# DataTunerX/datatunerx

Measured on AMD Instinct MI355X. Metric: tokens_per_sec_llama2_7b_lora_sft, higher is better.
Workload: dtype bf16; 1 GPU; model=llama2-7b, global_batch=64, seq_len=1024, parallelism=dp1, finetuning_type=lora

## Files before the change

datatunerx_amd/ops/hip/attn_bwd.hip:

```cpp
#include "dtx_common.h"

typedef __attribute__((ext_vector_type(16))) float f32x16;
typedef __attribute__((ext_vector_type(4))) unsigned int u32x4;

#define MFMA32(a, b, c) __builtin_amdgcn_mfma_f32_32x32x16_bf16(a, b, c, 0, 0, 0)
#define NEG_INF (-3.0e38f)
#define LOG2E 1.4426950408889634f

__device__ __forceinline__ unsigned bw_cvt_pk_bf16(float lo, float hi) {
  unsigned r;
  asm volatile("v_cvt_pk_bf16_f32 %0, %1, %2\n\ts_nop 1"
               : "=v"(r) : "v"(lo), "v"(hi));
  return r;
}

__device__ __forceinline__ int bw_crow(int r, int hi) {
  return (r & 3) + 8 * (r >> 2) + 4 * hi;
}

typedef __attribute__((ext_vector_type(4))) __bf16 bf16x4;
#define DTX_AS3 __attribute__((address_space(3)))
template <int STRIDE>
__device__ __forceinline__ short8v tr_bfrag(
    const DTX_AS3 unsigned short* img, int k0, int n0, int lane) {
  const int row = k0 + ((lane >> 2) & 3);
  const int col = n0 + ((lane >> 4) & 1) * 16 + (lane & 3) * 4;
  const DTX_AS3 unsigned short* p = img + row * STRIDE + col;
  union { bf16x4 v[2]; short8v s; } u;
  u.v[0] = __builtin_amdgcn_ds_read_tr16_b64_v4bf16(
      (DTX_AS3 bf16x4*)p);
  u.v[1] = __builtin_amdgcn_ds_read_tr16_b64_v4bf16(
      (DTX_AS3 bf16x4*)(p + 4 * STRIDE));
  return u.s;
}

__device__ __forceinline__ void conv_c_to_frag(const f32x16& p,
                                               short8v& f0, short8v& f1) {
  unsigned c0 = bw_cvt_pk_bf16(p[0], p[1]);
  unsigned c1 = bw_cvt_pk_bf16(p[2], p[3]);
  unsigned c2 = bw_cvt_pk_bf16(p[4], p[5]);
  unsigned c3 = bw_cvt_pk_bf16(p[6], p[7]);
  unsigned c4 = bw_cvt_pk_bf16(p[8], p[9]);
  unsigned c5 = bw_cvt_pk_bf16(p[10], p[11]);
  unsigned c6 = bw_cvt_pk_bf16(p[12], p[13]);
  unsigned c7 = bw_cvt_pk_bf16(p[14], p[15]);
  auto r02 = __builtin_amdgcn_permlane32_swap(c0, c2, false, false);
  auto r13 = __builtin_amdgcn_permlane32_swap(c1, c3, false, false);
  auto r46 = __builtin_amdgcn_permlane32_swap(c4, c6, false, false);
  auto r57 = __builtin_amdgcn_permlane32_swap(c5, c7, false, false);
  u32x4 lo{(unsigned)r02[0], (unsigned)r13[0],
           (unsigned)r02[1], (unsigned)r13[1]};
  u32x4 hi4{(unsigned)r46[0], (unsigned)r57[0],
            (unsigned)r46[1], (unsigned)r57[1]};
  f0 = *reinterpret_cast<short8v*>(&lo);
  f1 = *reinterpret_cast<short8v*>(&hi4);
}

template <int D>
__global__ __launch_bounds__(DTX_BLOCK)
void attn_delta2_kernel(const unsigned short* __restrict__ dO,
                        const unsigned short* __restrict__ O,
                        float* __restrict__ delta,
                        long nrows, int H, int S) {
  constexpr int LPR = D / 8;
  constexpr int RPW = 64 / LPR;
  const int lane = threadIdx.x & 63;
  const int wid = threadIdx.x >> 6;
  const int sub = lane / LPR;
  const int g = lane % LPR;
  for (long r0 = ((long)blockIdx.x * 4 + wid) * RPW; r0 < nrows;
       r0 += (long)gridDim.x * 4 * RPW) {
    const long row = r0 + sub;
    float acc = 0.f;
    if (row < nrows) {
      const long base = row * D + g * 8;
      float a[8], b8[8];
      load_bf16x8(dO + base, a);
      load_bf16x8(O + base, b8);
#pragma unroll
      for (int i = 0; i < 8; ++i) acc += a[i] * b8[i];
    }
#pragma unroll
    for (int off = LPR / 2; off > 0; off >>= 1)
      acc += __shfl_xor(acc, off, 64);
    if (g == 0 && row < nrows) {
      const int h = (int)(row % H);
      const long bs = row / H;
      const int s = (int)(bs % S);
      const long b = bs / S;
      delta[((long)b * H + h) * S + s] = acc;
    }
  }
}

template <int D>
struct DkdvLds {
  unsigned short Qr[2][64][D + 8];
  unsigned short dOr[2][64][D + 8];
};

template <int D>
__global__ __launch_bounds__(512, 1)
void attn_bwd_dkdv2_kernel(const unsigned short* __restrict__ Q,
                           const unsigned short* __restrict__ Kp,
                           const unsigned short* __restrict__ Vp,
                           const unsigned short* __restrict__ dO,
                           const float* __restrict__ lse_in,
                           const float* __restrict__ delta_in,
                           unsigned short* __restrict__ dK,
                           unsigned short* __restrict__ dV,
                           int B, int Hq, int Hkv, int S, int Skv,
                           float scale, int causal) {
  constexpr int DC16 = D / 16;
  constexpr int ND32 = D / 32;
  __shared__ DkdvLds<D> lds;
  __shared__ float lsed[2][64 + 64];

  const int lane = threadIdx.x & 63;
  const int wid = threadIdx.x >> 6;
  const int l31 = lane & 31;
  const int hi = lane >> 5;
  const int rep = Hq / Hkv;
  const bool role_dv = wid < 4;

  const int bh = blockIdx.y;
  const int b = bh / Hkv, hkv = bh % Hkv;
  const int kv0b = blockIdx.x * 128;
  const int kw = kv0b + (wid & 3) * 32;

  const int qrowstr = Hq * D, krowstr = Hkv * D;
  const long kbase = (long)b * Skv * krowstr + (long)hkv * D;
  const int diag = Skv - S;
  const float kscale = scale * LOG2E;

  short8v kfrag[DC16], vfrag[DC16];
  {
    const int krow = kw + l31;
#pragma unroll
    for (int kc = 0; kc < DC16; ++kc) {
      kfrag[kc] = short8v{0, 0, 0, 0, 0, 0, 0, 0};
      vfrag[kc] = short8v{0, 0, 0, 0, 0, 0, 0, 0};
      if (krow < Skv) {
        const long off = kbase + (long)krow * krowstr + kc * 16 + hi * 8;
        kfrag[kc] = *reinterpret_cast<const short8v*>(Kp + off);
        if (!role_dv)
          vfrag[kc] = *reinterpret_cast<const short8v*>(Vp + off);
      }
    }
  }

  f32x16 acc[ND32];
#pragma unroll
  for (int c = 0; c < ND32; ++c)
#pragma unroll
    for (int r = 0; r < 16; ++r) acc[c][r] = 0.f;

  for (int gi = 0; gi < rep; ++gi) {
    const int hq = hkv * rep + gi;
    const long qbase = (long)b * S * qrowstr + (long)hq * D;
    const long lbase = ((long)b * Hq + hq) * S;

    const int qs_lo = causal ? max(0, (kv0b - diag) / 64) : 0;
    const int qs_hi = (S + 63) / 64;
    constexpr int RIT = (64 * (D / 8)) / 512;
    short8v stg[RIT * 2];
    auto issue_stage = [&](int qs) {
#pragma unroll
      for (int it = 0; it < RIT; ++it) {
        const int idx = threadIdx.x + it * 512;
        const int row = idx / (D / 8), g = idx % (D / 8);
        const int q0s = qs * 64;
        short8v q8 = {0, 0, 0, 0, 0, 0, 0, 0};
        short8v d8 = {0, 0, 0, 0, 0, 0, 0, 0};
        if (q0s + row < S) {
          const long off = qbase + (long)(q0s + row) * qrowstr + g * 8;
          q8 = *reinterpret_cast<const short8v*>(Q + off);
          d8 = *reinterpret_cast<const short8v*>(dO + off);
        }
        stg[it * 2] = q8;
        stg[it * 2 + 1] = d8;
      }
    };
    auto write_stage = [&](int slot) {
#pragma unroll
      for (int it = 0; it < RIT; ++it) {
        const int idx = threadIdx.x + it * 512;
        const int row = idx / (D / 8), g = idx % (D / 8);
        *reinterpret_cast<short8v*>(&lds.Qr[slot][row][g * 8]) =
            stg[it * 2];
        *reinterpret_cast<short8v*>(&lds.dOr[slot][row][g * 8]) =
            stg[it * 2 + 1];
      }
    };
    auto write_lsed = [&](int slot, int qs) {
      if (threadIdx.x < 64) {
        const int qg = qs * 64 + threadIdx.x;
        lsed[slot][threadIdx.x] = qg < S ? lse_in[lbase + qg] : 0.f;
        lsed[slot][64 + threadIdx.x] =
            qg < S ? delta_in[lbase + qg] : 0.f;
      }
    };
    int cur = 0;
    if (qs_lo < qs_hi) {
      issue_stage(qs_lo);
      write_stage(0);
      write_lsed(0, qs_lo);
      __syncthreads();
    }
    for (int qs = qs_lo; qs < qs_hi; ++qs) {
      const int q0s = qs * 64;
      if (qs + 1 < qs_hi) issue_stage(qs + 1);

#pragma unroll
      for (int qh = 0; qh < 2; ++qh) {
      const int q0 = q0s + qh * 32;
      const int qoff = qh * 32;
      const bool live_tile =
          !(q0 >= S || (causal && (q0 + 31 + diag < kw)));
      if (live_tile) {

      f32x16 sv, dpv;
#pragma unroll
      for (int r = 0; r < 16; ++r) { sv[r] = 0.f; dpv[r] = 0.f; }
      if (role_dv) {
#pragma unroll
        for (int kc = 0; kc < DC16; ++kc) {
          short8v qa = *reinterpret_cast<const short8v*>(
              &lds.Qr[cur][qoff + l31][kc * 16 + hi * 8]);
          sv = MFMA32(qa, kfrag[kc], sv);
        }
      } else {
#pragma unroll
        for (int kc = 0; kc < DC16; ++kc) {
          short8v qa = *reinterpret_cast<const short8v*>(
              &lds.Qr[cur][qoff + l31][kc * 16 + hi * 8]);
          short8v da = *reinterpret_cast<const short8v*>(
              &lds.dOr[cur][qoff + l31][kc * 16 + hi * 8]);
          sv = MFMA32(qa, kfrag[kc], sv);
          dpv = MFMA32(da, vfrag[kc], dpv);
        }
      }

      const int kvg = kw + l31;
      const bool interior = (kv0b + 128 <= Skv) && (q0 + 32 <= S) &&
                            (!causal || (kw + 31 <= q0 + diag));
#pragma unroll
      for (int r = 0; r < 16; ++r) {
        const int qg = q0 + bw_crow(r, hi);
        const float lse2 = lsed[cur][qoff + bw_crow(r, hi)] * LOG2E;
        const float dlt = lsed[cur][64 + qoff + bw_crow(r, hi)];
        float p;
        if (interior) {
          p = __builtin_exp2f(sv[r] * kscale - lse2);
        } else {
          const bool dead = (kvg >= Skv) | (qg >= S) |
                            (causal && (kvg > qg + diag));
          p = dead ? 0.f : __builtin_exp2f(sv[r] * kscale - lse2);
        }
        sv[r] = p;
        dpv[r] = p * (dpv[r] - dlt) * scale;
      }

      short8v f0, f1;
      if (role_dv) conv_c_to_frag(sv, f0, f1);
      else conv_c_to_frag(dpv, f0, f1);
      const DTX_AS3 unsigned short* img3 = role_dv
          ? (const DTX_AS3 unsigned short*)&lds.dOr[cur][0][0]
          : (const DTX_AS3 unsigned short*)&lds.Qr[cur][0][0];
#pragma unroll
      for (int c = 0; c < ND32; ++c) {
        short8v b0 = tr_bfrag<D + 8>(img3, qoff + hi * 8, c * 32, lane);
        short8v b1 = tr_bfrag<D + 8>(img3, qoff + 16 + hi * 8, c * 32,
                                     lane);
        acc[c] = MFMA32(f0, b0, acc[c]);
        acc[c] = MFMA32(f1, b1, acc[c]);
        __builtin_amdgcn_sched_barrier(0);
      }
      }
      }
      if (qs + 1 < qs_hi) {
        write_stage(cur ^ 1);
        write_lsed(cur ^ 1, qs + 1);
      }
      __syncthreads();
      cur ^= 1;
    }
  }

  unsigned short* out = role_dv ? dV : dK;
#pragma unroll
  for (int r = 0; r < 16; ++r) {
    const int kvg = kw + bw_crow(r, hi);
    if (kvg < Skv) {
      unsigned short* orow = out + kbase + (long)kvg * krowstr;
#pragma unroll
      for (int c = 0; c < ND32; ++c)
        orow[c * 32 + l31] = f2bf(acc[c][r]);
    }
  }
}

template <int D>
struct DqLds {
  unsigned short K[2][128][D + 8];
  unsigned short V[2][128][D + 8];
};

template <int D>
__global__ __launch_bounds__(512, 1)
void attn_bwd_dq2_kernel(const unsigned short* __restrict__ Q,
                         const unsigned short* __restrict__ Kp,
                         const unsigned short* __restrict__ Vp,
                         const unsigned short* __restrict__ dO,
                         const float* __restrict__ lse_in,
                         const float* __restrict__ delta_in,
                         unsigned short* __restrict__ dQ,
                         int B, int Hq, int Hkv, int S, int Skv,
                         float scale, int causal) {
  constexpr int KVB = 64;
  constexpr int DC16 = D / 16;
  constexpr int ND32 = D / 32;
  __shared__ DqLds<D> lds;

  const int lane = threadIdx.x & 63;
  const int wid = threadIdx.x >> 6;
  const int l31 = lane & 31;
  const int hi = lane >> 5;

  const int bh = blockIdx.y;
  const int b = bh / Hq, hq = bh % Hq;
  const int hkv = hq / (Hq / Hkv);
  const int q0 = blockIdx.x * 256;
  const int qw = q0 + wid * 32;

  const int qrowstr = Hq * D, krowstr = Hkv * D;
  const long qbase = (long)b * S * qrowstr + (long)hq * D;
  const long kbase = (long)b * Skv * krowstr + (long)hkv * D;
  const long lbase = ((long)b * Hq + hq) * S;
  const int diag = Skv - S;
  const float kscale = scale * LOG2E;

  short8v qfrag[DC16], dofrag[DC16];
  float lse2 = 0.f, dlt = 0.f;
  {
    const int qrow = qw + l31;
    if (qrow < S) {
#pragma unroll
      for (int kc = 0; kc < DC16; ++kc) {
        const long off = qbase + (long)qrow * qrowstr + kc * 16 + hi * 8;
        qfrag[kc] = *reinterpret_cast<const short8v*>(Q + off);
        dofrag[kc] = *reinterpret_cast<const short8v*>(dO + off);
      }
      lse2 = lse_in[lbase + qrow] * LOG2E;
      dlt = delta_in[lbase + qrow];
    } else {
#pragma unroll
      for (int kc = 0; kc < DC16; ++kc) {
        qfrag[kc] = short8v{0, 0, 0, 0, 0, 0, 0, 0};
        dofrag[kc] = short8v{0, 0, 0, 0, 0, 0, 0, 0};
      }
    }
  }

  f32x16 dq_acc[ND32];
#pragma unroll
  for (int c = 0; c < ND32; ++c)
#pragma unroll
    for (int r = 0; r < 16; ++r) dq_acc[c][r] = 0.f;

  const int q_hi_blk = min(q0 + 255, S - 1);
  const int kv_hi = causal ? min(Skv - 1, q_hi_blk + diag) : (Skv - 1);
  const int nstages = kv_hi / 128 + 1;

  constexpr int KIT = (128 * (D / 8)) / 512;
  short8v stg[KIT * 2];
  auto issue_stage = [&](int st2) {
    const int kvs = st2 * 128;
#pragma unroll
    for (int it = 0; it < KIT; ++it) {
      const int idx = threadIdx.x + it * 512;
      const int row = idx / (D / 8), g = idx % (D / 8);
      short8v k8 = {0, 0, 0, 0, 0, 0, 0, 0};
      short8v v8 = {0, 0, 0, 0, 0, 0, 0, 0};
      if (kvs + row < Skv) {
        const long off = kbase + (long)(kvs + row) * krowstr + g * 8;
        k8 = *reinterpret_cast<const short8v*>(Kp + off);
        v8 = *reinterpret_cast<const short8v*>(Vp + off);
      }
      stg[it * 2] = k8;
      stg[it * 2 + 1] = v8;
    }
  };
  auto write_stage = [&](int slot) {
#pragma unroll
    for (int it = 0; it < KIT; ++it) {
      const int idx = threadIdx.x + it * 512;
      const int row = idx / (D / 8), g = idx % (D / 8);
      *reinterpret_cast<short8v*>(&lds.K[slot][row][g * 8]) =
          stg[it * 2];
      *reinterpret_cast<short8v*>(&lds.V[slot][row][g * 8]) =
          stg[it * 2 + 1];
    }
  };
  issue_stage(0);
  write_stage(0);
  __syncthreads();
  int cur = 0;
  for (int st2 = 0; st2 < nstages; ++st2) {
    if (st2 + 1 < nstages) issue_stage(st2 + 1);
    const int kvs = st2 * 128;

    for (int kh = 0; kh < 2; ++kh) {
    const int kv0 = kvs + kh * KVB;
    const int koff = kh * KVB;
    const bool wave_dead = (kv0 > kv_hi) ||
                           (causal && (kv0 > qw + 31 + diag));
    if (!wave_dead) {
      const int qg = qw + l31;
      const bool interior = (kv0 + KVB <= Skv) &&
                            (!causal || (kv0 + KVB - 1 <= qw + diag));
#pragma unroll
      for (int ss = 0; ss < 2; ++ss) {
        f32x16 st, dpt;
#pragma unroll
        for (int r = 0; r < 16; ++r) { st[r] = 0.f; dpt[r] = 0.f; }
#pragma unroll
        for (int kc = 0; kc < DC16; ++kc) {
          short8v ka = *reinterpret_cast<const short8v*>(
              &lds.K[cur][koff + ss * 32 + l31][kc * 16 + hi * 8]);
          short8v va = *reinterpret_cast<const short8v*>(
              &lds.V[cur][koff + ss * 32 + l31][kc * 16 + hi * 8]);
          st = MFMA32(ka, qfrag[kc], st);
          dpt = MFMA32(va, dofrag[kc], dpt);
        }
        f32x16 dst;
#pragma unroll
        for (int r = 0; r < 16; ++r) {
          float p;
          if (interior) {
            p = __builtin_exp2f(st[r] * kscale - lse2);
          } else {
            const int kvg = kv0 + ss * 32 + bw_crow(r, hi);
            const bool dead = (kvg >= Skv) | (qg >= S) |
                              (causal && (kvg > qg + diag));
            p = dead ? 0.f : __builtin_exp2f(st[r] * kscale - lse2);
          }
          dst[r] = p * (dpt[r] - dlt) * scale;
        }
        short8v f0, f1;
        conv_c_to_frag(dst, f0, f1);
        const DTX_AS3 unsigned short* k3 =
            (const DTX_AS3 unsigned short*)&lds.K[cur][0][0];
#pragma unroll
        for (int c = 0; c < ND32; ++c) {
          short8v kt0 = tr_bfrag<D + 8>(k3, koff + ss * 32 + hi * 8,
                                        c * 32, lane);
          dq_acc[c] = MFMA32(f0, kt0, dq_acc[c]);
        }
        __builtin_amdgcn_sched_barrier(0);
#pragma unroll
        for (int c = 0; c < ND32; ++c) {
          short8v kt1 = tr_bfrag<D + 8>(k3, koff + ss * 32 + 16 + hi * 8,
                                        c * 32, lane);
          dq_acc[c] = MFMA32(f1, kt1, dq_acc[c]);
        }
        __builtin_amdgcn_sched_barrier(0);
      }
    }
    }
    if (st2 + 1 < nstages) write_stage(cur ^ 1);
    __syncthreads();
    cur ^= 1;
  }

#pragma unroll
  for (int r = 0; r < 16; ++r) {
    const int qg = qw + bw_crow(r, hi);
    if (qg < S) {
      unsigned short* qrow = dQ + qbase + (long)qg * qrowstr;
#pragma unroll
      for (int c = 0; c < ND32; ++c)
        qrow[c * 32 + l31] = f2bf(dq_acc[c][r]);
    }
  }
}

void launch_attn_delta(const void* dO, const void* O, float* delta,
                       long nrows, int H, int S, int D, hipStream_t st) {
  const int rpw = 64 / (D / 8);
  long gw = DTX_CDIV(nrows, 4 * rpw);
  int grid = (int)(gw < 2048 ? (gw < 1 ? 1 : gw) : 2048);
  if (D == 128) {
    attn_delta2_kernel<128><<<grid, DTX_BLOCK, 0, st>>>(
        (const unsigned short*)dO, (const unsigned short*)O, delta,
        nrows, H, S);
  } else if (D == 64) {
    attn_delta2_kernel<64><<<grid, DTX_BLOCK, 0, st>>>(
        (const unsigned short*)dO, (const unsigned short*)O, delta,
        nrows, H, S);
  }
}

void launch_attn_bwd_dkdv(const void* q, const void* k, const void* v,
                          const void* dO, const float* lse,
                          const float* delta, void* dk, void* dv, int B,
                          int Hq, int Hkv, int S, int Skv, int D,
                          float scale, int causal, hipStream_t st) {
  dim3 grid(DTX_CDIV(Skv, 128), B * Hkv);
  if (D == 128) {
    attn_bwd_dkdv2_kernel<128><<<grid, 512, 0, st>>>(
        (const unsigned short*)q, (const unsigned short*)k,
        (const unsigned short*)v, (const unsigned short*)dO,
        lse, delta, (unsigned short*)dk, (unsigned short*)dv,
        B, Hq, Hkv, S, Skv, scale, causal);
  } else if (D == 64) {
    attn_bwd_dkdv2_kernel<64><<<grid, 512, 0, st>>>(
        (const unsigned short*)q, (const unsigned short*)k,
        (const unsigned short*)v, (const unsigned short*)dO,
        lse, delta, (unsigned short*)dk, (unsigned short*)dv,
        B, Hq, Hkv, S, Skv, scale, causal);
  }
}

void launch_attn_bwd_dq(const void* q, const void* k, const void* v,
                        const void* dO, const float* lse,
                        const float* delta, void* dq, int B, int Hq,
                        int Hkv, int S, int Skv, int D, float scale,
                        int causal, hipStream_t st) {
  dim3 grid(DTX_CDIV(S, 256), B * Hq);
  if (D == 128) {
    attn_bwd_dq2_kernel<128><<<grid, 512, 0, st>>>(
        (const unsigned short*)q, (const unsigned short*)k,
        (const unsigned short*)v,
        (const unsigned short*)dO, lse, delta, (unsigned short*)dq,
        B, Hq, Hkv, S, Skv, scale, causal);
  } else if (D == 64) {
    attn_bwd_dq2_kernel<64><<<grid, 512, 0, st>>>(
        (const unsigned short*)q, (const unsigned short*)k,
        (const unsigned short*)v,
        (const unsigned short*)dO, lse, delta, (unsigned short*)dq,
        B, Hq, Hkv, S, Skv, scale, causal);
  }
}
```

datatunerx_amd/ops/hip/bindings.cpp:

```cpp
#include <torch/extension.h>
#include <ATen/cuda/CUDAContext.h>
#include <hip/hip_runtime.h>

void launch_rmsnorm_fwd(const void*, const void*, void*, float*, int, int,
                        float, hipStream_t);
int rmsnorm_bwd_nblocks(int M);
void launch_rmsnorm_bwd(const void*, const void*, const void*, const float*,
                        const void*, void*, float*, float*, int, int,
                        hipStream_t);
void launch_rope(const void*, const float*, const float*, void*, long, int,
                 int, int, int, int, const int*, int, hipStream_t);
void launch_swiglu_fwd(const void*, const void*, void*, long, hipStream_t);
void launch_swiglu_bwd(const void*, const void*, const void*, void*, void*,
                       long, hipStream_t);
void launch_xent_fwd(const void*, const long*, float*, float*, long, int,
                     long, hipStream_t);
void launch_xent_bwd(const void*, const long*, const float*, const float*,
                     void*, long, int, long, hipStream_t);
void launch_dequant_int8(const void*, const float*, void*, long, int,
                         hipStream_t);
void launch_dequant_int4(const void*, const float*, void*, long, int, int,
                         hipStream_t);
void launch_xent_lse_merge(const void*, const long*, float*, float*,
                           float*, long, int, long, long, hipStream_t);
void launch_xent_dlogits(const void*, const long*, const float*, void*,
                         long, int, long, long, hipStream_t);
void launch_adamw(void*, float*, const float*, float*, float*, long, float,
                  float, float, float, float, int, hipStream_t);
void launch_l2_norm(const float*, float*, float*, long, hipStream_t);
int lora_contract_ksplit(int K, long M);
void launch_dropout_mask(void*, long, unsigned long long, float,
                         hipStream_t);
void launch_lora_contract(const void*, const void*, const void*, float*,
                          float*, long, int, int, unsigned long long,
                          float, hipStream_t);
void launch_lora_expand_add(void*, const float*, const void*, const void*,
                            long, int, int, float, unsigned long long,
                            float, hipStream_t);
int lora_wgrad_splitm(int K, int r, long M);
void launch_lora_wgrad(const float*, const void*, const void*, float*,
                       float*, long, int, int, float, unsigned long long,
                       float, hipStream_t);
void launch_attn_fwd(const void*, const void*, const void*, void*, float*,
                     int, int, int, int, int, int, float, int, hipStream_t);
void launch_transpose_sd(const void*, void*, int, int, int, int,
                         hipStream_t);
int attn_decode_nsplit(int Skv);
void launch_gemv_bf16(const void*, const void*, void*, int, int,
                      hipStream_t);
void launch_qgemv_int8(const void*, const void*, const float*, void*, int,
                       int, int, hipStream_t);
void launch_qgemv_int4(const void*, const void*, const float*, void*, int,
                       int, int, int, hipStream_t);
void launch_mlora_shrink(const void*, const void*, const int*, float*, int,
                         int, int, int, hipStream_t);
void launch_mlora_expand_add(void*, const float*, const void*, const float*,
                             const int*, int, int, int, int, hipStream_t);
void launch_gemm_nt(const void*, const void*, const void*, void*, long,
                    int, int, hipStream_t);
void launch_attn_decode(const void*, const void*, const void*,
                        const int*, float*, void*, float*, int, int, int,
                        int, int, float, int, hipStream_t);
void launch_attn_delta(const void*, const void*, float*, long, int, int,
                       int, hipStream_t);
void launch_attn_bwd_dkdv(const void*, const void*, const void*,
                          const void*, const float*, const float*,
                          void*, void*, int, int, int, int, int, int,
                          float, int, hipStream_t);
void launch_attn_bwd_dq(const void*, const void*, const void*,
                        const void*, const float*, const float*, void*,
                        int, int, int, int, int, int, float, int,
                        hipStream_t);

namespace {

hipStream_t cur_stream() {
  return (hipStream_t)at::cuda::getCurrentCUDAStream().stream();
}

void check_bf16_contig(const torch::Tensor& t, const char* name) {
  TORCH_CHECK(t.is_cuda(), name, " must be on GPU");
  TORCH_CHECK(t.scalar_type() == torch::kBFloat16, name, " must be bf16");
  TORCH_CHECK(t.is_contiguous(), name, " must be contiguous");
}

std::vector<torch::Tensor> rmsnorm_fwd(torch::Tensor x, torch::Tensor w,
                                       double eps) {
  check_bf16_contig(x, "x");
  check_bf16_contig(w, "w");
  const int H = (int)x.size(-1);
  const long M = x.numel() / H;
  TORCH_CHECK(H % 8 == 0, "H % 8");
  auto y = torch::empty_like(x);
  auto inv = torch::empty({M}, x.options().dtype(torch::kFloat));
  launch_rmsnorm_fwd(x.data_ptr(), w.data_ptr(), y.data_ptr(),
                     inv.data_ptr<float>(), (int)M, H, (float)eps,
                     cur_stream());
  return {y, inv};
}

std::vector<torch::Tensor> rmsnorm_bwd(torch::Tensor dy, torch::Tensor x,
                                       torch::Tensor w, torch::Tensor inv,
                                       c10::optional<torch::Tensor> dres) {
  check_bf16_contig(dy, "dy");
  check_bf16_contig(x, "x");
  const int H = (int)x.size(-1);
  const long M = x.numel() / H;
  auto dx = torch::empty_like(x);
  auto dw = torch::empty({H}, x.options().dtype(torch::kFloat));
  const int nb = rmsnorm_bwd_nblocks((int)M);
  auto part = torch::empty({nb, H}, x.options().dtype(torch::kFloat));
  const void* drp = nullptr;
  if (dres.has_value()) {
    check_bf16_contig(*dres, "dres");
    TORCH_CHECK(dres->numel() == x.numel(), "dres shape");
    drp = dres->data_ptr();
  }
  launch_rmsnorm_bwd(dy.data_ptr(), x.data_ptr(), w.data_ptr(),
                     inv.data_ptr<float>(), drp, dx.data_ptr(),
                     part.data_ptr<float>(), dw.data_ptr<float>(), (int)M, H,
                     cur_stream());
  return {dx, dw};
}

torch::Tensor rope(torch::Tensor x, torch::Tensor cosb, torch::Tensor sinb,
                   long pos0, bool backward,
                   c10::optional<torch::Tensor> pos_dev) {
  check_bf16_contig(x, "x");
  TORCH_CHECK(x.dim() == 4, "x must be [B,S,H,D]");
  TORCH_CHECK(cosb.scalar_type() == torch::kFloat && cosb.is_contiguous());
  const int B = (int)x.size(0), S = (int)x.size(1), H = (int)x.size(2),
            D = (int)x.size(3);
  TORCH_CHECK(D % 8 == 0, "D % 8");
  const int* pd = nullptr;
  int pos_per_b = 0;
  if (pos_dev.has_value()) {
    TORCH_CHECK(pos_dev->scalar_type() == torch::kInt &&
                pos_dev->is_cuda(), "pos_dev must be int32 on GPU");
    pd = pos_dev->data_ptr<int>();
    pos_per_b = pos_dev->numel() > 1;
    if (pos_per_b)
      TORCH_CHECK(pos_dev->numel() == B, "pos_dev must be [1] or [B]");
    TORCH_CHECK(cosb.size(0) >= S, "rope table too short");
  } else {
    TORCH_CHECK(cosb.size(0) >= pos0 + S, "rope table too short");
  }
  auto y = torch::empty_like(x);
  launch_rope(x.data_ptr(), cosb.data_ptr<float>(), sinb.data_ptr<float>(),
              y.data_ptr(), B, S, H, D, (int)pos0, backward ? 1 : 0, pd,
              pos_per_b, cur_stream());
  return y;
}

torch::Tensor swiglu_fwd(torch::Tensor gate, torch::Tensor up) {
  check_bf16_contig(gate, "gate");
  check_bf16_contig(up, "up");
  TORCH_CHECK(gate.numel() % 8 == 0);
  auto out = torch::empty_like(gate);
  launch_swiglu_fwd(gate.data_ptr(), up.data_ptr(), out.data_ptr(),
                    gate.numel(), cur_stream());
  return out;
}

std::vector<torch::Tensor> swiglu_bwd(torch::Tensor dout, torch::Tensor gate,
                                      torch::Tensor up) {
  check_bf16_contig(dout, "dout");
  auto dg = torch::empty_like(gate);
  auto du = torch::empty_like(up);
  launch_swiglu_bwd(dout.data_ptr(), gate.data_ptr(), up.data_ptr(),
                    dg.data_ptr(), du.data_ptr(), gate.numel(),
                    cur_stream());
  return {dg, du};
}

std::vector<torch::Tensor> xent_fwd(torch::Tensor logits,
                                    torch::Tensor targets, long ignore) {
  check_bf16_contig(logits, "logits");
  TORCH_CHECK(targets.scalar_type() == torch::kLong);
  const int V = (int)logits.size(-1);
  const long N = logits.numel() / V;
  TORCH_CHECK(V % 8 == 0, "V % 8");
  auto loss = torch::empty({N}, logits.options().dtype(torch::kFloat));
  auto lse = torch::empty({N}, logits.options().dtype(torch::kFloat));
  launch_xent_fwd(logits.data_ptr(), targets.data_ptr<long>(),
                  loss.data_ptr<float>(), lse.data_ptr<float>(), N, V,
                  ignore, cur_stream());
  return {loss, lse};
}

torch::Tensor xent_bwd(torch::Tensor logits, torch::Tensor targets,
                       torch::Tensor lse, torch::Tensor dloss, long ignore) {
  check_bf16_contig(logits, "logits");
  const int V = (int)logits.size(-1);
  const long N = logits.numel() / V;
  auto dlogits = torch::empty_like(logits);
  launch_xent_bwd(logits.data_ptr(), targets.data_ptr<long>(),
                  lse.data_ptr<float>(), dloss.data_ptr<float>(),
                  dlogits.data_ptr(), N, V, ignore, cur_stream());
  return dlogits;
}

static const void* opt_mask(const c10::optional<torch::Tensor>& m,
                            long numel, const char* name) {
  if (!m.has_value()) return nullptr;
  check_bf16_contig(*m, name);
  TORCH_CHECK(m->numel() == numel, name, " shape mismatch");
  return m->data_ptr();
}

torch::Tensor lora_contract(torch::Tensor x, torch::Tensor w,
                            c10::optional<torch::Tensor> mask,
                            int64_t seed, double keep) {
  check_bf16_contig(x, "x");
  check_bf16_contig(w, "w");
  const int K = (int)x.size(-1);
  const long M = x.numel() / K;
  const int r = (int)w.size(0);
  TORCH_CHECK(w.size(1) == K, "w [r,K] mismatch");
  TORCH_CHECK(r <= 64, "r <= 64");
  TORCH_CHECK(K % 8 == 0);
  auto t = torch::empty({M, r}, x.options().dtype(torch::kFloat));
  const int nsplit = lora_contract_ksplit(K, M);
  torch::Tensor part;
  float* part_ptr = nullptr;
  if (nsplit > 1) {
    part = torch::empty({nsplit, M, r}, x.options().dtype(torch::kFloat));
    part_ptr = part.data_ptr<float>();
  }
  launch_lora_contract(x.data_ptr(), w.data_ptr(),
                       opt_mask(mask, x.numel(), "mask"), part_ptr,
                       t.data_ptr<float>(), M, K, r,
                       (unsigned long long)seed, (float)keep,
                       cur_stream());
  return t;
}

void lora_expand_add(torch::Tensor y, torch::Tensor t, torch::Tensor w,
                     double scale, c10::optional<torch::Tensor> mask,
                     int64_t seed, double keep) {
  check_bf16_contig(y, "y");
  check_bf16_contig(w, "w");
  const int N = (int)y.size(-1);
  const long M = y.numel() / N;
  const int r = (int)w.size(1);
  TORCH_CHECK(w.size(0) == N, "w [N,r] mismatch");
  TORCH_CHECK(t.scalar_type() == torch::kFloat && t.is_contiguous());
  auto wt = w.t().contiguous();
  TORCH_CHECK(keep >= 1.0 || (r <= 16 && N % 8 == 0 && M >= 64),
              "RNG dropout needs the r<=16 fast path; materialize the "
              "mask for this shape");
  launch_lora_expand_add(y.data_ptr(), t.data_ptr<float>(), wt.data_ptr(),
                         opt_mask(mask, y.numel(), "mask"), M, N, r,
                         (float)scale, (unsigned long long)seed,
                         (float)keep, cur_stream());
}

torch::Tensor lora_wgrad(torch::Tensor t, torch::Tensor x, double scale,
                         c10::optional<torch::Tensor> mask,
                         int64_t seed, double keep) {
  check_bf16_contig(x, "x");
  TORCH_CHECK(t.scalar_type() == torch::kFloat && t.is_contiguous());
  const int K = (int)x.size(-1);
  const long M = x.numel() / K;
  const int r = (int)t.size(-1);
  auto out = torch::empty({r, K}, x.options().dtype(torch::kFloat));
  const int sm = lora_wgrad_splitm(K, r, M);
  auto part = torch::empty({sm, r, K}, x.options().dtype(torch::kFloat));
  launch_lora_wgrad(t.data_ptr<float>(), x.data_ptr(),
                    opt_mask(mask, x.numel(), "mask"),
                    part.data_ptr<float>(), out.data_ptr<float>(), M, K, r,
                    (float)scale, (unsigned long long)seed, (float)keep,
                    cur_stream());
  return out;
}

torch::Tensor dropout_mask(int64_t M, int64_t K, int64_t seed, double keep,
                           torch::Tensor like) {
  TORCH_CHECK((M * K) % 8 == 0, "M*K % 8 == 0");
  auto m = torch::empty({M, K}, like.options().dtype(torch::kBFloat16));
  launch_dropout_mask(m.data_ptr(), M * K, (unsigned long long)seed,
                      (float)keep, cur_stream());
  return m;
}

void adamw(torch::Tensor p, torch::Tensor master, torch::Tensor grad,
           torch::Tensor m, torch::Tensor v, double lr, double b1, double b2,
           double eps, double wd, long step) {
  check_bf16_contig(p, "p");
  TORCH_CHECK(master.scalar_type() == torch::kFloat);
  TORCH_CHECK(grad.scalar_type() == torch::kFloat);
  TORCH_CHECK(p.numel() % 4 == 0, "flat param buffer must be padded to 4");
  launch_adamw(p.data_ptr(), master.data_ptr<float>(),
               grad.data_ptr<float>(), m.data_ptr<float>(),
               v.data_ptr<float>(), p.numel(), (float)lr, (float)b1,
               (float)b2, (float)eps, (float)wd, (int)step, cur_stream());
}

torch::Tensor l2_norm(torch::Tensor x) {
  TORCH_CHECK(x.is_cuda() && x.scalar_type() == torch::kFloat &&
              x.is_contiguous());
  auto ws = torch::empty({1024}, x.options());
  auto out = torch::empty({1}, x.options());
  launch_l2_norm(x.data_ptr<float>(), ws.data_ptr<float>(),
                 out.data_ptr<float>(), x.numel(), cur_stream());
  return out;
}

torch::Tensor transpose_sd(torch::Tensor x) {
  check_bf16_contig(x, "x");
  TORCH_CHECK(x.dim() == 4, "x must be [B,S,H,D]");
  const int B = (int)x.size(0), S = (int)x.size(1), H = (int)x.size(2),
            D = (int)x.size(3);
  auto xt = torch::empty({B, H, D, S}, x.options());
  launch_transpose_sd(x.data_ptr(), xt.data_ptr(), B, S, H, D,
                      cur_stream());
  return xt;
}

std::vector<torch::Tensor> attn_fwd(torch::Tensor q, torch::Tensor k,
                                    torch::Tensor v, bool causal,
                                    double scale) {
  check_bf16_contig(q, "q");
  check_bf16_contig(k, "k");
  check_bf16_contig(v, "v");
  const int B = (int)q.size(0), S = (int)q.size(1), Hq = (int)q.size(2),
            D = (int)q.size(3);
  const int Skv = (int)k.size(1), Hkv = (int)k.size(2);
  TORCH_CHECK(v.size(1) == Skv && v.size(2) == Hkv && v.size(3) == D,
              "v must be BSHD like k");
  TORCH_CHECK(D == 64 || D == 128, "D must be 64 or 128");
  TORCH_CHECK(Hq % Hkv == 0, "GQA group");
  auto o = torch::empty_like(q);
  auto lse = torch::empty({B, Hq, S}, q.options().dtype(torch::kFloat));
  launch_attn_fwd(q.data_ptr(), k.data_ptr(), v.data_ptr(), o.data_ptr(),
                  lse.data_ptr<float>(), B, Hq, Hkv, S, Skv, D,
                  (float)scale, causal ? 1 : 0, cur_stream());
  return {o, lse};
}

torch::Tensor gemm_nt(torch::Tensor a, torch::Tensor b,
                      c10::optional<torch::Tensor> src) {
  check_bf16_contig(a, "a");
  check_bf16_contig(b, "b");
  const int K = (int)b.size(1), N = (int)b.size(0);
  const long M = a.numel() / K;
  TORCH_CHECK(a.size(-1) == K, "gemm_nt: inner dims");
  TORCH_CHECK(N % 256 == 0 && K % 64 == 0 && K >= 128,
              "gemm_nt: unsupported shape N=", N, " K=", K);
  auto sizes = a.sizes().vec();
  sizes[sizes.size() - 1] = N;
  auto c = torch::empty(sizes, a.options());
  const void* sp = nullptr;
  if (src.has_value()) {
    check_bf16_contig(*src, "src");
    TORCH_CHECK(src->numel() == M * N, "gemm_nt: src shape");
    sp = src->data_ptr();
  }
  launch_gemm_nt(a.data_ptr(), b.data_ptr(), sp, c.data_ptr(), M, N, K,
                 cur_stream());
  return c;
}

torch::Tensor dequant_int8(torch::Tensor q, torch::Tensor scale) {
  TORCH_CHECK(q.is_cuda() && q.scalar_type() == torch::kChar &&
              q.is_contiguous());
  const int K = (int)q.size(1);
  const long N = q.size(0);
  TORCH_CHECK(K % 8 == 0, "K % 8");
  auto out = torch::empty({N, K},
                          q.options().dtype(torch::kBFloat16));
  launch_dequant_int8(q.data_ptr(), scale.data_ptr<float>(),
                      out.data_ptr(), N, K, cur_stream());
  return out;
}

torch::Tensor dequant_int4(torch::Tensor packed, torch::Tensor scale,
                           long group) {
  TORCH_CHECK(packed.is_cuda() && packed.scalar_type() == torch::kByte &&
              packed.is_contiguous());
  const int K = (int)packed.size(1) * 2;
  const long N = packed.size(0);
  TORCH_CHECK(K % 8 == 0 && group % 8 == 0, "K/group alignment");
  auto out = torch::empty({N, K},
                          packed.options().dtype(torch::kBFloat16));
  launch_dequant_int4(packed.data_ptr(), scale.data_ptr<float>(),
                      out.data_ptr(), N, K, (int)group, cur_stream());
  return out;
}

void xent_lse_merge(torch::Tensor logits, torch::Tensor targets,
                    torch::Tensor m_run, torch::Tensor l_run,
                    torch::Tensor tgt, long v0, long ignore_index) {
  check_bf16_contig(logits, "logits");
  const int Vc = (int)logits.size(-1);
  const long N = logits.numel() / Vc;
  TORCH_CHECK(Vc % 8 == 0, "Vc % 8");
  launch_xent_lse_merge(logits.data_ptr(), targets.data_ptr<long>(),
                        m_run.data_ptr<float>(), l_run.data_ptr<float>(),
                        tgt.data_ptr<float>(), N, Vc, v0, ignore_index,
                        cur_stream());
}

torch::Tensor xent_dlogits(torch::Tensor logits, torch::Tensor targets,
                           torch::Tensor lse, long v0, long ignore_index) {
  check_bf16_contig(logits, "logits");
  const int Vc = (int)logits.size(-1);
  const long N = logits.numel() / Vc;
  TORCH_CHECK(Vc % 8 == 0, "Vc % 8");
  auto dl = torch::empty_like(logits);
  launch_xent_dlogits(logits.data_ptr(), targets.data_ptr<long>(),
                      lse.data_ptr<float>(), dl.data_ptr(), N, Vc, v0,
                      ignore_index, cur_stream());
  return dl;
}

torch::Tensor gemv(torch::Tensor x, torch::Tensor w) {
  check_bf16_contig(x, "x");
  check_bf16_contig(w, "w");
  const int K = (int)w.size(1), N = (int)w.size(0);
  TORCH_CHECK(x.numel() == K, "gemv wants a single row");
  TORCH_CHECK(K % 8 == 0, "K % 8");
  auto sizes = x.sizes().vec();
  sizes[sizes.size() - 1] = N;
  auto y = torch::empty(sizes, x.options());
  launch_gemv_bf16(x.data_ptr(), w.data_ptr(), y.data_ptr(), N, K,
                   cur_stream());
  return y;
}

static torch::Tensor qgemv_out(const torch::Tensor& x, int N) {
  auto sizes = x.sizes().vec();
  sizes[sizes.size() - 1] = N;
  return torch::empty(sizes, x.options());
}

static long qgemv_rows(const torch::Tensor& x, int K) {
  check_bf16_contig(x, "x");
  TORCH_CHECK(x.dim() >= 1 && x.size(-1) == K, "qgemv: x inner dim != K");
  const long M = x.numel() / K;
  TORCH_CHECK(M >= 1 && M <= 16, "qgemv: 1 <= M <= 16, got ", M);
  TORCH_CHECK((uintptr_t)x.data_ptr() % 16 == 0, "qgemv: x 16-B aligned");
  return M;
}

static void qgemv_check_w(const torch::Tensor& w, at::ScalarType dt,
                          const torch::Tensor& scale, long nscale) {
  TORCH_CHECK(w.is_cuda() && w.scalar_type() == dt && w.dim() == 2 &&
              w.is_contiguous(), "qgemv: weight dtype/layout");
  TORCH_CHECK((uintptr_t)w.data_ptr() % 16 == 0,
              "qgemv: weight 16-B aligned");
  TORCH_CHECK(scale.is_cuda() && scale.scalar_type() == torch::kFloat &&
              scale.is_contiguous() && scale.numel() == nscale,
              "qgemv: scale dtype/shape");
}

torch::Tensor qgemv_int8(torch::Tensor x, torch::Tensor q,
                         torch::Tensor scale) {
  const int N = (int)q.size(0), K = (int)q.size(1);
  TORCH_CHECK(K > 0 && K % 16 == 0, "qgemv_int8: K % 16");
  qgemv_check_w(q, torch::kChar, scale, N);
  const long M = qgemv_rows(x, K);
  auto y = qgemv_out(x, N);
  launch_qgemv_int8(x.data_ptr(), q.data_ptr(), scale.data_ptr<float>(),
                    y.data_ptr(), (int)M, N, K, cur_stream());
  return y;
}

torch::Tensor qgemv_int4(torch::Tensor x, torch::Tensor packed,
                         torch::Tensor scale, long group) {
  const int N = (int)packed.size(0), K = (int)packed.size(1) * 2;
  TORCH_CHECK(K > 0 && K % 32 == 0, "qgemv_int4: K % 32");
  TORCH_CHECK(group > 0 && group % 32 == 0 && K % group == 0,
              "qgemv_int4: group % 32, K % group");
  qgemv_check_w(packed, torch::kByte, scale, (long)N * (K / group));
  const long M = qgemv_rows(x, K);
  auto y = qgemv_out(x, N);
  launch_qgemv_int4(x.data_ptr(), packed.data_ptr(),
                    scale.data_ptr<float>(), y.data_ptr(), (int)M, N, K,
                    (int)group, cur_stream());
  return y;
}

void mlora_add(torch::Tensor y, torch::Tensor x, torch::Tensor A,
               torch::Tensor Bt, torch::Tensor scale, torch::Tensor idx) {
  check_bf16_contig(y, "y");
  check_bf16_contig(x, "x");
  check_bf16_contig(A, "A");
  check_bf16_contig(Bt, "Bt");
  TORCH_CHECK(y.dim() == 2 && x.dim() == 2 && A.dim() == 3 && Bt.dim() == 3,
              "mlora: y [M,N], x [M,K], A [G,R,K], Bt [G,R,N]");
  const long M = x.size(0), K = x.size(1), N = y.size(1);
  const long G = A.size(0), R = A.size(1);
  TORCH_CHECK(y.size(0) == M, "mlora: y/x rows differ");
  TORCH_CHECK(A.size(2) == K && Bt.size(0) == G && Bt.size(1) == R &&
              Bt.size(2) == N, "mlora: A [G,R,K] / Bt [G,R,N] mismatch");
  TORCH_CHECK(M >= 1 && M <= 16, "mlora: 1 <= M <= 16, got ", M);
  TORCH_CHECK(K >= 8 && K % 8 == 0 && N >= 8 && N % 8 == 0,
              "mlora: K % 8, N % 8");
  TORCH_CHECK(R == 8 || R == 16 || R == 32 || R == 64,
              "mlora: R must be 8, 16, 32 or 64, got ", R);
  TORCH_CHECK(G >= 1 && G * R * std::max(K, N) < (1L << 40),
              "mlora: stack size");
  TORCH_CHECK(scale.is_cuda() && scale.scalar_type() == torch::kFloat &&
              scale.is_contiguous() && scale.numel() == G,
              "mlora: scale must be f32 [G] on the GPU");
  TORCH_CHECK(idx.is_cuda() && idx.scalar_type() == torch::kInt &&
              idx.is_contiguous() && idx.numel() == M,
              "mlora: idx must be int32 [M] on the GPU");
  TORCH_CHECK((uintptr_t)y.data_ptr() % 16 == 0 &&
              (uintptr_t)x.data_ptr() % 16 == 0 &&
              (uintptr_t)A.data_ptr() % 16 == 0 &&
              (uintptr_t)Bt.data_ptr() % 16 == 0, "mlora: 16-B alignment");
  auto t = torch::empty({M, R}, x.options().dtype(torch::kFloat));
  launch_mlora_shrink(x.data_ptr(), A.data_ptr(), idx.data_ptr<int>(),
                      t.data_ptr<float>(), (int)M, (int)K, (int)R, (int)G,
                      cur_stream());
  launch_mlora_expand_add(y.data_ptr(), t.data_ptr<float>(), Bt.data_ptr(),
                          scale.data_ptr<float>(), idx.data_ptr<int>(),
                          (int)M, (int)N, (int)R, (int)G, cur_stream());
}

std::vector<torch::Tensor> attn_decode(torch::Tensor q, torch::Tensor k,
                                       torch::Tensor v, double scale,
                                       c10::optional<torch::Tensor>
                                           len_dev) {
  check_bf16_contig(q, "q");
  const int B = (int)q.size(0), Hq = (int)q.size(2), D = (int)q.size(3);
  const int Skv = (int)k.size(1), Hkv = (int)k.size(2);
  auto dense_kv = [&](const torch::Tensor& t, const char* n) {
    TORCH_CHECK(t.is_cuda() && t.scalar_type() == torch::kBFloat16,
                n, " must be bf16 GPU");
    TORCH_CHECK(t.stride(3) == 1 && t.stride(2) == D &&
                t.stride(1) == (long)Hkv * D,
                n, " must be s/h/d-dense");
    if (B > 1) TORCH_CHECK(t.is_contiguous(), n, " batch>1 needs contig");
  };
  dense_kv(k, "k");
  dense_kv(v, "v");
  TORCH_CHECK(q.size(1) == 1, "decode path wants S == 1");
  TORCH_CHECK(D == 64 || D == 128, "D must be 64 or 128");
  const int ns = attn_decode_nsplit(Skv);
  auto part = torch::empty({(long)B * Hq, ns, D + 2},
                           q.options().dtype(torch::kFloat));
  auto o = torch::empty_like(q);
  auto lse = torch::empty({B, Hq, 1}, q.options().dtype(torch::kFloat));
  const int* ld = nullptr;
  int len_stride = 0;
  if (len_dev.has_value()) {
    TORCH_CHECK(len_dev->scalar_type() == torch::kInt &&
                len_dev->is_cuda(), "len_dev must be int32 on GPU");
    ld = len_dev->data_ptr<int>();
    len_stride = len_dev->numel() > 1;
    if (len_stride)
      TORCH_CHECK(len_dev->numel() == B, "len_dev must be [1] or [B]");
  }
  launch_attn_decode(q.data_ptr(), k.data_ptr(), v.data_ptr(), ld,
                     part.data_ptr<float>(), o.data_ptr(),
                     lse.data_ptr<float>(), B, Hq, Hkv, Skv, D,
                     (float)scale, len_stride, cur_stream());
  return {o, lse};
}

std::vector<torch::Tensor> attn_bwd(torch::Tensor q, torch::Tensor k,
                                    torch::Tensor v, torch::Tensor o,
                                    torch::Tensor dO, torch::Tensor lse,
                                    bool causal, double scale) {
  check_bf16_contig(q, "q");
  check_bf16_contig(k, "k");
  check_bf16_contig(v, "v");
  auto dO_c = dO.contiguous();
  const int B = (int)q.size(0), S = (int)q.size(1), Hq = (int)q.size(2),
            D = (int)q.size(3);
  const int Skv = (int)k.size(1), Hkv = (int)k.size(2);
  auto delta = torch::empty({B, Hq, S}, q.options().dtype(torch::kFloat));
  launch_attn_delta(dO_c.data_ptr(), o.data_ptr(), delta.data_ptr<float>(),
                    (long)B * S * Hq, Hq, S, D, cur_stream());
  auto dq = torch::empty_like(q);
  auto dk = torch::empty_like(k);
  auto dv = torch::empty_like(v);
  launch_attn_bwd_dkdv(q.data_ptr(), k.data_ptr(), v.data_ptr(),
                       dO_c.data_ptr(), lse.data_ptr<float>(),
                       delta.data_ptr<float>(), dk.data_ptr(),
                       dv.data_ptr(), B, Hq, Hkv, S, Skv, D,
                       (float)scale, causal ? 1 : 0, cur_stream());
  launch_attn_bwd_dq(q.data_ptr(), k.data_ptr(), v.data_ptr(),
                     dO_c.data_ptr(), lse.data_ptr<float>(),
                     delta.data_ptr<float>(), dq.data_ptr(), B, Hq, Hkv, S,
                     Skv, D, (float)scale, causal ? 1 : 0, cur_stream());
  return {dq, dk, dv};
}

}

PYBIND11_MODULE(TORCH_EXTENSION_NAME, m) {
  m.def("rmsnorm_fwd", &rmsnorm_fwd);
  m.def("rmsnorm_bwd", &rmsnorm_bwd, py::arg("dy"), py::arg("x"),
        py::arg("w"), py::arg("inv"), py::arg("dres") = py::none());
  m.def("rope", &rope, py::arg("x"), py::arg("cosb"), py::arg("sinb"),
        py::arg("pos0"), py::arg("backward"),
        py::arg("pos_dev") = py::none());
  m.def("swiglu_fwd", &swiglu_fwd);
  m.def("swiglu_bwd", &swiglu_bwd);
  m.def("xent_fwd", &xent_fwd);
  m.def("xent_bwd", &xent_bwd);
  m.def("xent_lse_merge", &xent_lse_merge);
  m.def("dequant_int8", &dequant_int8);
  m.def("dequant_int4", &dequant_int4);
  m.def("xent_dlogits", &xent_dlogits);
  m.def("lora_contract", &lora_contract, py::arg("x"), py::arg("w"),
        py::arg("mask") = py::none(), py::arg("seed") = 0,
        py::arg("keep") = 1.0);
  m.def("lora_expand_add", &lora_expand_add, py::arg("y"), py::arg("t"),
        py::arg("w"), py::arg("scale"), py::arg("mask") = py::none(),
        py::arg("seed") = 0, py::arg("keep") = 1.0);
  m.def("lora_wgrad", &lora_wgrad, py::arg("t"), py::arg("x"),
        py::arg("scale"), py::arg("mask") = py::none(),
        py::arg("seed") = 0, py::arg("keep") = 1.0);
  m.def("dropout_mask", &dropout_mask, py::arg("m"), py::arg("k"),
        py::arg("seed"), py::arg("keep"), py::arg("like"));
  m.def("adamw", &adamw);
  m.def("l2_norm", &l2_norm);
  m.def("attn_fwd", &attn_fwd);
  m.def("attn_bwd", &attn_bwd);
  m.def("transpose_sd", &transpose_sd);
  m.def("gemv", &gemv);
  m.def("qgemv_int8", &qgemv_int8, py::arg("x"), py::arg("q"),
        py::arg("scale"));
  m.def("qgemv_int4", &qgemv_int4, py::arg("x"), py::arg("packed"),
        py::arg("scale"), py::arg("group") = 64);
  m.def("mlora_add", &mlora_add, py::arg("y"), py::arg("x"), py::arg("A"),
        py::arg("Bt"), py::arg("scale"), py::arg("idx"));
  m.def("gemm_nt", &gemm_nt, py::arg("a"), py::arg("b"),
        py::arg("src") = py::none());
  m.def("attn_decode", &attn_decode, py::arg("q"), py::arg("k"),
        py::arg("v"), py::arg("scale"), py::arg("len_dev") = py::none());
}
```

Baseline: 35150 tokens/s.

## Fuse attention-backward delta computation into dQ kernel and streamline dK/dV staging

The separate delta kernel (rowsum of dO*O) is removed. The dQ kernel now loads O alongside dO, computes delta in registers and writes it out, so it runs before the dK/dV kernel. The dK/dV kernel loads LSE and delta per stage through two waves with prescaled LSE, and reads them from LDS as vector loads. Bounds checks become clamped addresses plus selects, which lets loads stay unconditional. This saves one kernel launch and one extra pass over dO, at the cost of extra O traffic in dQ and unconditional V loads for every wave.

```diff
diff --git a/datatunerx_amd/ops/hip/attn_bwd.hip b/datatunerx_amd/ops/hip/attn_bwd.hip
--- a/datatunerx_amd/ops/hip/attn_bwd.hip
+++ b/datatunerx_amd/ops/hip/attn_bwd.hip
@@ -2,6 +2,7 @@
 
 typedef __attribute__((ext_vector_type(16))) float f32x16;
 typedef __attribute__((ext_vector_type(4))) unsigned int u32x4;
+typedef __attribute__((ext_vector_type(4))) float f32x4;
 
 #define MFMA32(a, b, c) __builtin_amdgcn_mfma_f32_32x32x16_bf16(a, b, c, 0, 0, 0)
 #define NEG_INF (-3.0e38f)
@@ -57,43 +58,6 @@
 }
 
 template <int D>
-__global__ __launch_bounds__(DTX_BLOCK)
-void attn_delta2_kernel(const unsigned short* __restrict__ dO,
-                        const unsigned short* __restrict__ O,
-                        float* __restrict__ delta,
-                        long nrows, int H, int S) {
-  constexpr int LPR = D / 8;
-  constexpr int RPW = 64 / LPR;
-  const int lane = threadIdx.x & 63;
-  const int wid = threadIdx.x >> 6;
-  const int sub = lane / LPR;
-  const int g = lane % LPR;
-  for (long r0 = ((long)blockIdx.x * 4 + wid) * RPW; r0 < nrows;
-       r0 += (long)gridDim.x * 4 * RPW) {
-    const long row = r0 + sub;
-    float acc = 0.f;
-    if (row < nrows) {
-      const long base = row * D + g * 8;
-      float a[8], b8[8];
-      load_bf16x8(dO + base, a);
-      load_bf16x8(O + base, b8);
-#pragma unroll
-      for (int i = 0; i < 8; ++i) acc += a[i] * b8[i];
-    }
-#pragma unroll
-    for (int off = LPR / 2; off > 0; off >>= 1)
-      acc += __shfl_xor(acc, off, 64);
-    if (g == 0 && row < nrows) {
-      const int h = (int)(row % H);
-      const long bs = row / H;
-      const int s = (int)(bs % S);
-      const long b = bs / S;
-      delta[((long)b * H + h) * S + s] = acc;
-    }
-  }
-}
-
-template <int D>
 struct DkdvLds {
   unsigned short Qr[2][64][D + 8];
   unsigned short dOr[2][64][D + 8];
@@ -114,14 +78,15 @@
   constexpr int DC16 = D / 16;
   constexpr int ND32 = D / 32;
   __shared__ DkdvLds<D> lds;
-  __shared__ float lsed[2][64 + 64];
+  __shared__ __attribute__((aligned(16))) float lsed[2][64 + 64];
 
   const int lane = threadIdx.x & 63;
-  const int wid = threadIdx.x >> 6;
+  const int wid = __builtin_amdgcn_readfirstlane(threadIdx.x >> 6);
   const int l31 = lane & 31;
   const int hi = lane >> 5;
   const int rep = Hq / Hkv;
   const bool role_dv = wid < 4;
+  const short8v zero8 = {0, 0, 0, 0, 0, 0, 0, 0};
 
   const int bh = blockIdx.y;
   const int b = bh / Hkv, hkv = bh % Hkv;
@@ -136,16 +101,17 @@
   short8v kfrag[DC16], vfrag[DC16];
   {
     const int krow = kw + l31;
+    const bool kok = krow < Skv;
+    const long off0 =
+        kbase + (long)min(krow, Skv - 1) * krowstr + hi * 8;
 #pragma unroll
     for (int kc = 0; kc < DC16; ++kc) {
-      kfrag[kc] = short8v{0, 0, 0, 0, 0, 0, 0, 0};
-      vfrag[kc] = short8v{0, 0, 0, 0, 0, 0, 0, 0};
-      if (krow < Skv) {
-        const long off = kbase + (long)krow * krowstr + kc * 16 + hi * 8;
-        kfrag[kc] = *reinterpret_cast<const short8v*>(Kp + off);
-        if (!role_dv)
-          vfrag[kc] = *reinterpret_cast<const short8v*>(Vp + off);
-      }
+      const short8v k8 =
+          *reinterpret_cast<const short8v*>(Kp + off0 + kc * 16);
+      const short8v v8 =
+          *reinterpret_cast<const short8v*>(Vp + off0 + kc * 16);
+      kfrag[kc] = kok ? k8 : zero8;
+      vfrag[kc] = kok ? v8 : zero8;
     }
   }
 
@@ -164,47 +130,42 @@
     const int qs_hi = (S + 63) / 64;
     constexpr int RIT = (64 * (D / 8)) / 512;
     short8v stg[RIT * 2];
+    float lsv;
     auto issue_stage = [&](int qs) {
+      const int q0s = qs * 64;
 #pragma unroll
       for (int it = 0; it < RIT; ++it) {
         const int idx = threadIdx.x + it * 512;
         const int row = idx / (D / 8), g = idx % (D / 8);
-        const int q0s = qs * 64;
-        short8v q8 = {0, 0, 0, 0, 0, 0, 0, 0};
-        short8v d8 = {0, 0, 0, 0, 0, 0, 0, 0};
-        if (q0s + row < S) {
-          const long off = qbase + (long)(q0s + row) * qrowstr + g * 8;
-          q8 = *reinterpret_cast<const short8v*>(Q + off);
-          d8 = *reinterpret_cast<const short8v*>(dO + off);
-        }
-        stg[it * 2] = q8;
-        stg[it * 2 + 1] = d8;
-      }
+        const long off =
+            qbase + (long)min(q0s + row, S - 1) * qrowstr + g * 8;
+        stg[it * 2] = *reinterpret_cast<const short8v*>(Q + off);
+        stg[it * 2 + 1] = *reinterpret_cast<const short8v*>(dO + off);
+      }
+      const float* src = (wid & 1) ? delta_in : lse_in;
+      lsv = src[lbase + min(q0s + lane, S - 1)];
     };
-    auto write_stage = [&](int slot) {
+    auto write_stage = [&](int slot, int qs) {
+      const int q0s = qs * 64;
 #pragma unroll
       for (int it = 0; it < RIT; ++it) {
         const int idx = threadIdx.x + it * 512;
         const int row = idx / (D / 8), g = idx % (D / 8);
+        const bool ok = q0s + row < S;
         *reinterpret_cast<short8v*>(&lds.Qr[slot][row][g * 8]) =
-            stg[it * 2];
+            ok ? stg[it * 2] : zero8;
         *reinterpret_cast<short8v*>(&lds.dOr[slot][row][g * 8]) =
-            stg[it * 2 + 1];
-      }
-    };
-    auto write_lsed = [&](int slot, int qs) {
-      if (threadIdx.x < 64) {
-        const int qg = qs * 64 + threadIdx.x;
-        lsed[slot][threadIdx.x] = qg < S ? lse_in[lbase + qg] : 0.f;
-        lsed[slot][64 + threadIdx.x] =
-            qg < S ? delta_in[lbase + qg] : 0.f;
+            ok ? stg[it * 2 + 1] : zero8;
+      }
+      if (wid < 2) {
+        const float x = q0s + lane < S ? lsv : 0.f;
+        lsed[slot][wid * 64 + lane] = wid ? x : x * LOG2E;
       }
     };
     int cur = 0;
     if (qs_lo < qs_hi) {
       issue_stage(qs_lo);
-      write_stage(0);
-      write_lsed(0, qs_lo);
+      write_stage(0, qs_lo);
       __syncthreads();
     }
     for (int qs = qs_lo; qs < qs_hi; ++qs) {
@@ -218,6 +179,12 @@
       const bool live_tile =
           !(q0 >= S || (causal && (q0 + 31 + diag < kw)));
       if (live_tile) {
+
+      f32x4 l4[4], d4[4];
+#pragma unroll
+      for (int g = 0; g < 4; ++g)
+        l4[g] = *reinterpret_cast<const f32x4*>(
+            &lsed[cur][qoff + 8 * g + 4 * hi]);
 
       f32x16 sv, dpv;
 #pragma unroll
@@ -241,29 +208,37 @@
         }
       }
 
-      const int kvg = kw + l31;
       const bool interior = (kv0b + 128 <= Skv) && (q0 + 32 <= S) &&
                             (!causal || (kw + 31 <= q0 + diag));
-#pragma unroll
-      for (int r = 0; r < 16; ++r) {
-        const int qg = q0 + bw_crow(r, hi);
-        const float lse2 = lsed[cur][qoff + bw_crow(r, hi)] * LOG2E;
-        const float dlt = lsed[cur][64 + qoff + bw_crow(r, hi)];
-        float p;
-        if (interior) {
-          p = __builtin_exp2f(sv[r] * kscale - lse2);
-        } else {
+      if (interior) {
+#pragma unroll
+        for (int r = 0; r < 16; ++r)
+          sv[r] = __builtin_exp2f(sv[r] * kscale - l4[r >> 2][r & 3]);
+      } else {
+        const int kvg = kw + l31;
+#pragma unroll
+        for (int r = 0; r < 16; ++r) {
+          const int qg = q0 + bw_crow(r, hi);
           const bool dead = (kvg >= Skv) | (qg >= S) |
                             (causal && (kvg > qg + diag));
-          p = dead ? 0.f : __builtin_exp2f(sv[r] * kscale - lse2);
-        }
-        sv[r] = p;
-        dpv[r] = p * (dpv[r] - dlt) * scale;
+          sv[r] = dead ? 0.f
+                       : __builtin_exp2f(sv[r] * kscale - l4[r >> 2][r & 3]);
+        }
       }
 
       short8v f0, f1;
-      if (role_dv) conv_c_to_frag(sv, f0, f1);
-      else conv_c_to_frag(dpv, f0, f1);
+      if (role_dv) {
+        conv_c_to_frag(sv, f0, f1);
+      } else {
+#pragma unroll
+        for (int g = 0; g < 4; ++g)
+          d4[g] = *reinterpret_cast<const f32x4*>(
+              &lsed[cur][64 + qoff + 8 * g + 4 * hi]);
+#pragma unroll
+        for (int r = 0; r < 16; ++r)
+          dpv[r] = sv[r] * (dpv[r] - d4[r >> 2][r & 3]) * scale;
+        conv_c_to_frag(dpv, f0, f1);
+      }
       const DTX_AS3 unsigned short* img3 = role_dv
           ? (const DTX_AS3 unsigned short*)&lds.dOr[cur][0][0]
           : (const DTX_AS3 unsigned short*)&lds.Qr[cur][0][0];
@@ -278,10 +253,7 @@
       }
       }
       }
-      if (qs + 1 < qs_hi) {
-        write_stage(cur ^ 1);
-        write_lsed(cur ^ 1, qs + 1);
-      }
+      if (qs + 1 < qs_hi) write_stage(cur ^ 1, qs + 1);
       __syncthreads();
       cur ^= 1;
     }
@@ -312,8 +284,9 @@
                          const unsigned short* __restrict__ Kp,
                          const unsigned short* __restrict__ Vp,
                          const unsigned short* __restrict__ dO,
+                         const unsigned short* __restrict__ O,
                          const float* __restrict__ lse_in,
-                         const float* __restrict__ delta_in,
+                         float* __restrict__ delta_out,
                          unsigned short* __restrict__ dQ,
                          int B, int Hq, int Hkv, int S, int Skv,
                          float scale, int causal) {
@@ -345,14 +318,27 @@
   {
     const int qrow = qw + l31;
     if (qrow < S) {
+      float part[DC16];
 #pragma unroll
       for (int kc = 0; kc < DC16; ++kc) {
         const long off = qbase + (long)qrow * qrowstr + kc * 16 + hi * 8;
         qfrag[kc] = *reinterpret_cast<const short8v*>(Q + off);
         dofrag[kc] = *reinterpret_cast<const short8v*>(dO + off);
-      }
+        const short8v o8 = *reinterpret_cast<const short8v*>(O + off);
+        float acc = 0.f;
+#pragma unroll
+        for (int j = 0; j < 8; ++j)
+          acc += bf2f((unsigned short)dofrag[kc][j]) *
+                 bf2f((unsigned short)o8[j]);
+        part[kc] = acc;
+      }
+#pragma unroll
+      for (int w = DC16 / 2; w > 0; w >>= 1)
+#pragma unroll
+        for (int kc = 0; kc < w; ++kc) part[kc] += part[kc + w];
       lse2 = lse_in[lbase + qrow] * LOG2E;
-      dlt = delta_in[lbase + qrow];
+      dlt = part[0] + __shfl_xor(part[0], 32, 64);
+      if (hi == 0) delta_out[lbase + qrow] = dlt;
     } else {
 #pragma unroll
       for (int kc = 0; kc < DC16; ++kc) {
@@ -482,22 +468,6 @@
       for (int c = 0; c < ND32; ++c)
         qrow[c * 32 + l31] = f2bf(dq_acc[c][r]);
     }
-  }
-}
-
-void launch_attn_delta(const void* dO, const void* O, float* delta,
-                       long nrows, int H, int S, int D, hipStream_t st) {
-  const int rpw = 64 / (D / 8);
-  long gw = DTX_CDIV(nrows, 4 * rpw);
-  int grid = (int)(gw < 2048 ? (gw < 1 ? 1 : gw) : 2048);
-  if (D == 128) {
-    attn_delta2_kernel<128><<<grid, DTX_BLOCK, 0, st>>>(
-        (const unsigned short*)dO, (const unsigned short*)O, delta,
-        nrows, H, S);
-  } else if (D == 64) {
-    attn_delta2_kernel<64><<<grid, DTX_BLOCK, 0, st>>>(
-        (const unsigned short*)dO, (const unsigned short*)O, delta,
-        nrows, H, S);
   }
 }
 
@@ -523,22 +493,22 @@
 }
 
 void launch_attn_bwd_dq(const void* q, const void* k, const void* v,
-                        const void* dO, const float* lse,
-                        const float* delta, void* dq, int B, int Hq,
+                        const void* dO, const void* o, const float* lse,
+                        float* delta, void* dq, int B, int Hq,
                         int Hkv, int S, int Skv, int D, float scale,
                         int causal, hipStream_t st) {
   dim3 grid(DTX_CDIV(S, 256), B * Hq);
   if (D == 128) {
     attn_bwd_dq2_kernel<128><<<grid, 512, 0, st>>>(
         (const unsigned short*)q, (const unsigned short*)k,
-        (const unsigned short*)v,
-        (const unsigned short*)dO, lse, delta, (unsigned short*)dq,
+        (const unsigned short*)v, (const unsigned short*)dO,
+        (const unsigned short*)o, lse, delta, (unsigned short*)dq,
         B, Hq, Hkv, S, Skv, scale, causal);
   } else if (D == 64) {
     attn_bwd_dq2_kernel<64><<<grid, 512, 0, st>>>(
         (const unsigned short*)q, (const unsigned short*)k,
-        (const unsigned short*)v,
-        (const unsigned short*)dO, lse, delta, (unsigned short*)dq,
+        (const unsigned short*)v, (const unsigned short*)dO,
+        (const unsigned short*)o, lse, delta, (unsigned short*)dq,
         B, Hq, Hkv, S, Skv, scale, causal);
   }
 }
diff --git a/datatunerx_amd/ops/hip/bindings.cpp b/datatunerx_amd/ops/hip/bindings.cpp
--- a/datatunerx_amd/ops/hip/bindings.cpp
+++ b/datatunerx_amd/ops/hip/bindings.cpp
@@ -61,15 +61,13 @@
 void launch_attn_decode(const void*, const void*, const void*,
                         const int*, float*, void*, float*, int, int, int,
                         int, int, float, int, hipStream_t);
-void launch_attn_delta(const void*, const void*, float*, long, int, int,
-                       int, hipStream_t);
 void launch_attn_bwd_dkdv(const void*, const void*, const void*,
                           const void*, const float*, const float*,
                           void*, void*, int, int, int, int, int, int,
                           float, int, hipStream_t);
 void launch_attn_bwd_dq(const void*, const void*, const void*,
-                        const void*, const float*, const float*, void*,
-                        int, int, int, int, int, int, float, int,
+                        const void*, const void*, const float*, float*,
+                        void*, int, int, int, int, int, int, float, int,
                         hipStream_t);
 
 namespace {
@@ -572,21 +570,20 @@
   const int B = (int)q.size(0), S = (int)q.size(1), Hq = (int)q.size(2),
             D = (int)q.size(3);
   const int Skv = (int)k.size(1), Hkv = (int)k.size(2);
+  check_bf16_contig(o, "o");
   auto delta = torch::empty({B, Hq, S}, q.options().dtype(torch::kFloat));
-  launch_attn_delta(dO_c.data_ptr(), o.data_ptr(), delta.data_ptr<float>(),
-                    (long)B * S * Hq, Hq, S, D, cur_stream());
   auto dq = torch::empty_like(q);
   auto dk = torch::empty_like(k);
   auto dv = torch::empty_like(v);
+  launch_attn_bwd_dq(q.data_ptr(), k.data_ptr(), v.data_ptr(),
+                     dO_c.data_ptr(), o.data_ptr(), lse.data_ptr<float>(),
+                     delta.data_ptr<float>(), dq.data_ptr(), B, Hq, Hkv, S,
+                     Skv, D, (float)scale, causal ? 1 : 0, cur_stream());
   launch_attn_bwd_dkdv(q.data_ptr(), k.data_ptr(), v.data_ptr(),
                        dO_c.data_ptr(), lse.data_ptr<float>(),
                        delta.data_ptr<float>(), dk.data_ptr(),
                        dv.data_ptr(), B, Hq, Hkv, S, Skv, D,
                        (float)scale, causal ? 1 : 0, cur_stream());
-  launch_attn_bwd_dq(q.data_ptr(), k.data_ptr(), v.data_ptr(),
-                     dO_c.data_ptr(), lse.data_ptr<float>(),
-                     delta.data_ptr<float>(), dq.data_ptr(), B, Hq, Hkv, S,
-                     Skv, D, (float)scale, causal ? 1 : 0, cur_stream());
   return {dq, dk, dv};
 }
 
```

Result: faster. 36440 tokens/s, median of 6 (+3.7%).
